# buctcurry/ICKA

Hardware: AMD Instinct MI355X
Metric: MNER samples/sec (fwd+bwd) at seq=128, 36 regions, bs=32 per GPU (higher is better)
Workload: dtype bf16; 1 GPU; c2: bert(H768,L12,h12,I3072)+36x2048 regions, seq_len 128, per-GPU batch 32, 1 cross layer(s), gated head, 13 labels, train mode p=0.1, token-CE loss; global_batch=32, seq_len=128, regions=36, parallelism=dp1, launch=hipgraph, precision=bf16, accumulate=1

## Files before the change

icka_amd/csrc/fusion.hip:

```cpp
#include <math.h>

#include "common.h"

namespace {

__device__ __forceinline__ void ld8(const bf16_t* p, float (&o)[8]) {
    const bf16x8 v = as_bf16x8(*reinterpret_cast<const u32x4*>(p));
#pragma unroll
    for (int e = 0; e < 8; ++e) o[e] = bf2f(v[e]);
}
__device__ __forceinline__ void st8(bf16_t* p, const float (&v)[8]) {
    bf16x8 o;
#pragma unroll
    for (int e = 0; e < 8; ++e) o[e] = f2bf(v[e]);
    *reinterpret_cast<u32x4*>(p) = as_u32x4(o);
}
__device__ __forceinline__ float block_sum(float v, float* red) {
    v = wave_sum(v);
    const int w = threadIdx.x >> 6;
    if ((threadIdx.x & 63) == 0) red[w] = v;
    __syncthreads();
    float t = 0.f;
    for (int i = 0; i < (int)(blockDim.x >> 6); ++i) t += red[i];
    __syncthreads();
// ... 261 lines not shown
                       (const bf16_t*)seq, lds, (const bf16_t*)cross, ldc, dW, dbias, B, S, H, accumulate);
    ICKA_CHECK_LAUNCH();
    return 0;
}


namespace {

constexpr int CLS_TB = 16;
constexpr int CLS_MAXC = 16;

__device__ __forceinline__ void cls_ld8(const bf16_t* p, float (&o)[8]) {
    const bf16x8 v = as_bf16x8(*reinterpret_cast<const u32x4*>(p));
#pragma unroll
    for (int e = 0; e < 8; ++e) o[e] = bf2f(v[e]);
}
__device__ __forceinline__ void cls_st8(bf16_t* p, const float (&v)[8]) {
    bf16x8 o;
#pragma unroll
    for (int e = 0; e < 8; ++e) o[e] = f2bf(v[e]);
    *reinterpret_cast<u32x4*>(p) = as_u32x4(o);
}

template <bool F16>
__global__ __launch_bounds__(256) void cls_head_fwd_kernel(const bf16_t* __restrict__ seq, const bf16_t* __restrict__ gated,
                                                           const bf16_t* __restrict__ W, const float* __restrict__ bias,
                                                           float* __restrict__ logits, int M, int H, int C) {
    extern __shared__ __attribute__((aligned(16))) char cls_smem[];
    __shared__ float s_red[4][CLS_MAXC][65];
    bf16_t* sW = reinterpret_cast<bf16_t*>(cls_smem);
    const int tid = threadIdx.x, lane = tid & 63, wave = tid >> 6;
    const int nch = (2 * H) >> 3, hch = H >> 3;
    for (int i = tid; i < C * nch; i += 256)
        *reinterpret_cast<u32x4*>(sW + (int64_t)i * 8) = *reinterpret_cast<const u32x4*>(W + (int64_t)i * 8);
    __syncthreads();
    const int nw = gridDim.x * 4;
    for (int row0 = (blockIdx.x * 4 + wave) * 2; row0 < M; row0 += 2 * nw) {
        u32x4 xr[2][4];
#pragma unroll
        for (int r = 0; r < 2; ++r)
#pragma unroll
            for (int i = 0; i < 4; ++i) {
                const int j = lane + 64 * i, row = row0 + r;
                xr[r][i] = u32x4{0u, 0u, 0u, 0u};
                if (j < nch && row < M)
                    xr[r][i] = *reinterpret_cast<const u32x4*>(j < hch ? seq + (int64_t)row * H + j * 8
                                                                       : gated + (int64_t)row * H + (j - hch) * 8);
            }
        float acc[2][CLS_MAXC];
#pragma unroll
        for (int r = 0; r < 2; ++r)
#pragma unroll
            for (int c = 0; c < CLS_MAXC; ++c) acc[r][c] = 0.f;
#pragma unroll
        for (int i = 0; i < 4; ++i) {
            const int j = lane + 64 * i;
            if (j < nch) {
#pragma unroll
                for (int c = 0; c < CLS_MAXC; ++c) {
                    if (c < C) {
                        float w[8];
                        if constexpr (F16) {
                            const f16x8 wv = __builtin_bit_cast(f16x8, *reinterpret_cast<const u32x4*>(sW + (int64_t)c * 2 * H + j * 8));
#pragma unroll
                            for (int e = 0; e < 8; ++e) w[e] = (float)wv[e];
                        } else {
                            cls_ld8(sW + (int64_t)c * 2 * H + j * 8, w);
                        }
#pragma unroll
                        for (int r = 0; r < 2; ++r) {
                            if constexpr (F16) {
// ... 94 lines not shown
            } else {
                const bf16x8 gv = as_bf16x8(gr[u]), cv = as_bf16x8(cr4[u]);
                float uu[8], dc[8];
#pragma unroll
                for (int e = 0; e < 8; ++e) {
                    const float g = bf2f(gv[e]);
                    uu[e] = dx[e] * bf2f(cv[e]) * g * (1.f - g);
                    dc[e] = dx[e] * g;
                }
                cls_st8(du + row * H + h, uu);
                cls_st8(dcross + row * H + h, dc);
            }
        }
    }
#pragma unroll
    for (int c = 0; c < CC; ++c)
        if (c < C) {
            float* p = myslab + (int64_t)c * 2 * H + j * 8;
            *reinterpret_cast<f32x4*>(p) = f32x4{dW[c][0], dW[c][1], dW[c][2], dW[c][3]};
            *reinterpret_cast<f32x4*>(p + 4) = f32x4{dW[c][4], dW[c][5], dW[c][6], dW[c][7]};
        }
}

}

extern "C" int32_t icka_cls_head_bwd_slabs(int32_t M) { return (M + CLS_TB - 1) / CLS_TB; }
extern "C" int64_t icka_cls_head_slab_floats(int32_t H, int32_t C) { return (int64_t)C * 2 * H + CLS_MAXC; }

static int cls_head_fwd_impl(bool f16, const void* seq, const void* gated, const void* W, const float* bias, float* logits,
                             int32_t M, int32_t H, int32_t C, void* stream) {
    if (!seq || !gated || !W || !logits) return ICKA_E_ARG;
    if (M <= 0 || H <= 0 || H % 8 || C <= 0 || C > CLS_MAXC || 2 * H / 8 > 256 || (int64_t)C * 2 * H * 2 > 44 * 1024)
        return ICKA_E_SHAPE;
    if ((reinterpret_cast<uintptr_t>(seq) | reinterpret_cast<uintptr_t>(gated) | reinterpret_cast<uintptr_t>(W)) & 15)
        return ICKA_E_ALIGN;
    int grid = (M + 7) / 8;
    grid = grid > 512 ? 512 : grid;
    if (f16)
        hipLaunchKernelGGL(cls_head_fwd_kernel<true>, dim3(grid), dim3(256), (size_t)C * 2 * H * 2, (hipStream_t)stream,
                           (const bf16_t*)seq, (const bf16_t*)gated, (const bf16_t*)W, bias, logits, M, H, C);
    else
        hipLaunchKernelGGL(cls_head_fwd_kernel<false>, dim3(grid), dim3(256), (size_t)C * 2 * H * 2, (hipStream_t)stream,
                           (const bf16_t*)seq, (const bf16_t*)gated, (const bf16_t*)W, bias, logits, M, H, C);
    ICKA_CHECK_LAUNCH();
    return 0;
}
extern "C" int icka_cls_head_fwd(const void* seq, const void* gated, const void* W, const float* bias, float* logits,
                                 int32_t M, int32_t H, int32_t C, void* stream) {
    return cls_head_fwd_impl(false, seq, gated, W, bias, logits, M, H, C, stream);
}
extern "C" int icka_cls_head_fwd_h(const void* seq, const void* gated, const void* W, const float* bias, float* logits,
                                   int32_t M, int32_t H, int32_t C, void* stream) {
    return cls_head_fwd_impl(true, seq, gated, W, bias, logits, M, H, C, stream);
}

extern "C" int icka_cls_head_bwd(const void* dl, int64_t ldd, const void* seq, const void* gated, const void* gate,
                                 const void* cross, const void* W, void* dseq, void* du, void* dcross, float* partials,
                                 int32_t M, int32_t H, int32_t C, void* stream) {
    if (!dl || !seq || !gated || !gate || !cross || !W || !dseq || !du || !dcross || !partials) return ICKA_E_ARG;
    if (M <= 0 || H <= 0 || H % 8 || C <= 0 || C > CLS_MAXC || 2 * H / 8 > 256 || ldd < C) return ICKA_E_SHAPE;
    const uintptr_t al = reinterpret_cast<uintptr_t>(seq) | reinterpret_cast<uintptr_t>(gated) |
                         reinterpret_cast<uintptr_t>(gate) | reinterpret_cast<uintptr_t>(cross) |
                         reinterpret_cast<uintptr_t>(W) | reinterpret_cast<uintptr_t>(dseq) |
                         reinterpret_cast<uintptr_t>(du) | reinterpret_cast<uintptr_t>(dcross) |
                         reinterpret_cast<uintptr_t>(partials);
    if (al & 15) return ICKA_E_ALIGN;
    const int grid = icka_cls_head_bwd_slabs(M);
    if (C <= 13)
        hipLaunchKernelGGL((cls_head_bwd_kernel<13>), dim3(grid), dim3(256), 0, (hipStream_t)stream,
                           (const bf16_t*)dl, ldd, (const bf16_t*)seq, (const bf16_t*)gated, (const bf16_t*)gate,
                           (const bf16_t*)cross, (const bf16_t*)W, (bf16_t*)dseq, (bf16_t*)du, (bf16_t*)dcross,
                           partials, M, H, C);
    else
        hipLaunchKernelGGL((cls_head_bwd_kernel<CLS_MAXC>), dim3(grid), dim3(256), 0, (hipStream_t)stream,
                           (const bf16_t*)dl, ldd, (const bf16_t*)seq, (const bf16_t*)gated, (const bf16_t*)gate,
                           (const bf16_t*)cross, (const bf16_t*)W, (bf16_t*)dseq, (bf16_t*)du, (bf16_t*)dcross,
                           partials, M, H, C);
    ICKA_CHECK_LAUNCH();
    return 0;
}
```

icka_amd/csrc/layernorm.hip:

```cpp
#include "common.h"
#include "ln_row.h"
#include <cstdlib>

namespace {

constexpr int BWD_BLOCKS = 1024;
constexpr int SLOTS = 4;

template <int NCH>
__global__ __launch_bounds__(256) void ln_fwd_kernel(const LnFwdArgs a_) {
    LnFwdArgs a = a_;
    a.drop = drop_resolve(a.drop);
    const int lane = threadIdx.x & 63;
    const int wid = blockIdx.x * 4 + (threadIdx.x >> 6), nw = gridDim.x * 4;
    ln_fwd_rows<NCH>(a, wid, nw, a.M, lane);
}

struct LnBwdArgs {
    const bf16_t* dy; int64_t lddy; const bf16_t* dy2; int64_t lddy2; const bf16_t* xhat; const float* rstd;
    const float* gamma; bf16_t* dres; int64_t lddres; bf16_t* dx; int64_t lddx; float* partials;
    int M, H; DropCfg drop;
    uint8_t* row_live; uint8_t* row_live_kv; const float* add_mask; int mask_S;
};

// ... 192 lines not shown
}
__global__ __launch_bounds__(256) void ln_cols_kernel(const bf16_t* __restrict__ dy, int64_t lddy,
                                                      const bf16_t* __restrict__ dy2, int64_t lddy2,
                                                      const bf16_t* __restrict__ xhat, const bf16_t* __restrict__ dx,
                                                      int64_t lddx, float* __restrict__ partials, int M, int H,
                                                      int rows_per_group) {
    ln_cols_body(dy, lddy, dy2, lddy2, xhat, dx, lddx, partials, M, H, rows_per_group, blockIdx.x, blockIdx.y);
}

struct LnColsArgs {
    int nx, groups, rows_per_group;
};
template <int NCH, bool LIVE = false>
__global__ __launch_bounds__(256) void ln_bwd_fused_kernel(const LnBwdArgs a, const LnColsArgs c) {
    const int ncol = c.nx * c.groups;
    if ((int)blockIdx.x >= ncol) {
        ln_rows_body<NCH, LIVE>(a, blockIdx.x - ncol, gridDim.x - ncol);
        return;
    }
    ln_cols_body(a.dy, a.lddy, a.dy2, a.lddy2, a.xhat, nullptr, 0, a.partials, a.M, a.H, c.rows_per_group,
                 blockIdx.x % c.nx, blockIdx.x / c.nx);
}

__global__ __launch_bounds__(1024) void finalize_kernel(const float* __restrict__ partials, int nslab, int H, float* o0,
                                                        float* o1, float* o2, float* o3, int accumulate) {
    __shared__ float red[16][64];
    const int cx = threadIdx.x & 63, sy = threadIdx.x >> 6;
    const int idx = blockIdx.x * 64 + cx;
    float s = 0.f;
    if (idx < SLOTS * H) {
        const int slot = idx / H, c = idx - slot * H;
        for (int b = sy; b < nslab; b += 16) s += partials[((int64_t)b * SLOTS + slot) * H + c];
    }
    red[sy][cx] = s;
    __syncthreads();
    if (sy == 0 && idx < SLOTS * H) {
        const int slot = idx / H, c = idx - slot * H;
        float* out = slot == 0 ? o0 : slot == 1 ? o1 : slot == 2 ? o2 : o3;
        if (out) {
            float t = 0.f;
#pragma unroll
            for (int k = 0; k < 16; ++k) t += red[k][cx];
            out[c] = accumulate ? out[c] + t : t;
        }
    }
}

struct EmbFwdArgs {
    const int64_t* ids; const int64_t* tt; const float* word; const float* pos; const float* type;
    const float* gamma; const float* beta; bf16_t* y; void* yf; bf16_t* xhat; float* rstd;
    int M, S, H, vocab, n_type; float eps; DropCfg drop;
    const int32_t* src; const bf16_t* prompt; int S_in, P, pos_offset;
    int yf_f16;
};

template <int NCH>
__global__ __launch_bounds__(256) void embed_fwd_kernel(const EmbFwdArgs a_) {
    EmbFwdArgs a = a_;
    a.drop = drop_resolve(a.drop);
    const int lane = threadIdx.x & 63;
    const int wid = blockIdx.x * 4 + (threadIdx.x >> 6), nw = gridDim.x * 4;
    const int nchunk = a.H >> 3;
    const float inv_h = 1.f / (float)a.H;
    for (int row = wid; row < a.M; row += nw) {
        const int sp = row % a.S;
        const int sidx = a.src ? a.src[sp] : sp;
        const bf16_t* prow = sidx < 0 ? a.prompt + ((int64_t)(row / a.S) * a.P + (-1 - sidx)) * a.H : nullptr;
// ... 36 lines not shown
                float g[8], b[8], xh[8], o[8];
                load8f(a.gamma + c * 8, g);
                load8f(a.beta + c * 8, b);
                const uint32_t base = (uint32_t)row * (uint32_t)a.H + c * 8;
#pragma unroll
                for (int e = 0; e < 8; ++e) {
                    xh[e] = (s[i][e] - mean) * rstd;
                    o[e] = (g[e] * xh[e] + b[e]) * drop_mul(a.drop, base + e);
                }
                store8(a.y + (int64_t)row * a.H + c * 8, o);
                if (a.yf) store8t(a.yf, a.yf_f16, (int64_t)row * a.H + c * 8, o);
                if (a.xhat) store8(a.xhat + (int64_t)row * a.H + c * 8, xh);
            }
        }
    }
}

struct EmbBwdArgs {
    const bf16_t* dy; const int64_t* ids; const int64_t* tt; const bf16_t* xhat; const float* rstd;
    const float* gamma; float* dword; float* dpos; float* dtype; float* partials;
    int M, S, H, vocab, n_type, padding_idx; DropCfg drop;
    const int32_t* src; bf16_t* dprompt; int S_in, P, pos_offset;
    float* dtok;
};

template <int NCH>
__global__ __launch_bounds__(256) void embed_bwd_kernel(const EmbBwdArgs a_) {
    EmbBwdArgs a = a_;
    a.drop = drop_resolve(a.drop);
    extern __shared__ __attribute__((aligned(16))) float lds_f[];
    const int lane = threadIdx.x & 63;
    const int wid = blockIdx.x * 4 + (threadIdx.x >> 6), nw = gridDim.x * 4;
    const int nchunk = a.H >> 3;
    const float inv_h = 1.f / (float)a.H;
    float acc[4][NCH][8];
#pragma unroll
    for (int s = 0; s < 4; ++s)
#pragma unroll
        for (int i = 0; i < NCH; ++i)
#pragma unroll
            for (int e = 0; e < 8; ++e) acc[s][i][e] = 0.f;

    for (int row = wid; row < a.M; row += nw) {
        int64_t id = a.ids[row];
        id = id < 0 ? 0 : (id >= a.vocab ? a.vocab - 1 : id);
        int64_t t = a.tt ? a.tt[row] : 0;
// ... 38 lines not shown
                    }
                }
            }
        }
        __builtin_amdgcn_wave_barrier();
        for (int j = lane; j < a.H; j += 64) {
            const float ds = rowbuf[j];
            if (a.dtok) a.dtok[(int64_t)row * a.H + j] = id != a.padding_idx ? ds : 0.f;
            else if (id != a.padding_idx) atomicAdd(a.dword + id * a.H + j, ds);
            atomicAdd(a.dpos + (int64_t)sp * a.H + j, ds);
            if (a.n_type > 2) atomicAdd(a.dtype + t * a.H + j, ds);
        }
        __builtin_amdgcn_wave_barrier();
    }
    flush_columns<NCH, 4>(acc, lds_f, a.partials, a.H);
}

template <int NCH>
__global__ __launch_bounds__(512) void embed_bwd_pos_kernel(const EmbBwdArgs a_) {
    EmbBwdArgs a = a_;
    a.drop = drop_resolve(a.drop);
    extern __shared__ __attribute__((aligned(16))) float lds_f[];
    const int tid = threadIdx.x, lane = tid & 63, wave = tid >> 6;
    const int sp = blockIdx.x, B = a.M / a.S;
    const int nchunk = a.H >> 3;
    const float inv_h = 1.f / (float)a.H;
    float acc[5][NCH][8];
#pragma unroll
    for (int s = 0; s < 5; ++s)
#pragma unroll
        for (int i = 0; i < NCH; ++i)
#pragma unroll
            for (int e = 0; e < 8; ++e) acc[s][i][e] = 0.f;
    float* rowbuf = lds_f + wave * a.H;

    const int sidx = a.src ? a.src[sp] : sp;
    for (int b = wave; b < B; b += 8) {
        const int row = b * a.S + sp;
        int64_t id = sidx < 0 ? 0 : a.ids[a.src ? (int64_t)b * a.S_in + sidx : row];
        id = id < 0 ? 0 : (id >= a.vocab ? a.vocab - 1 : id);
        int64_t t = a.tt ? a.tt[row] : 0;
        t = t < 0 ? 0 : (t >= a.n_type ? a.n_type - 1 : t);
        float xh[NCH][8], gd[NCH][8];
        float s1 = 0.f, s2 = 0.f;
#pragma unroll
        for (int i = 0; i < NCH; ++i) {
            const int c = lane + 64 * i;
            if (c < nchunk) {
                float dy[8], g[8];
                load8(a.dy + (int64_t)row * a.H + c * 8, dy);
                load8(a.xhat + (int64_t)row * a.H + c * 8, xh[i]);
                load8f(a.gamma + c * 8, g);
                const uint32_t base = (uint32_t)row * (uint32_t)a.H + c * 8;
#pragma unroll
                for (int e = 0; e < 8; ++e) {
                    const float dl = dy[e] * drop_mul(a.drop, base + e);
                    gd[i][e] = g[e] * dl;
                    s1 += gd[i][e];
                    s2 += gd[i][e] * xh[i][e];
                    acc[0][i][e] += dl * xh[i][e];
// ... 32 lines not shown
                const float ds = rowbuf[j];
                if (id != a.padding_idx) atomicAdd(a.dword + id * a.H + j, ds);
                if (a.n_type > 2) atomicAdd(a.dtype + t * a.H + j, ds);
            }
        }
        __builtin_amdgcn_wave_barrier();
    }
#pragma unroll
    for (int s = 0; s < 5; ++s) {
        __syncthreads();
#pragma unroll
        for (int i = 0; i < NCH; ++i) {
            const int c = lane + 64 * i;
            if (c < nchunk) {
#pragma unroll
                for (int e = 0; e < 8; ++e) rowbuf[c * 8 + e] = acc[s][i][e];
            }
        }
        __syncthreads();
        for (int j = tid; j < a.H; j += 512) {
            float v = 0.f;
#pragma unroll
            for (int w = 0; w < 8; ++w) v += lds_f[w * a.H + j];
            if (s < 4) a.partials[((int64_t)sp * SLOTS + s) * a.H + j] = v;
            else a.dpos[(int64_t)(sp + a.pos_offset) * a.H + j] += v;
        }
    }
}

inline int pick_nch(int H) { return (H / 8 + 63) / 64; }
inline int rows_knob(const char* name, int dflt) {
    const char* e = getenv(name);
    const int v = e ? atoi(e) : 0;
    return v >= 1 && v <= 16 ? v : dflt;
}
const int kLnRowsEnv = rows_knob("ICKA_TUNE_LN_ROWS_PER_WAVE", 0);
const int kLnBwdRowsEnv = rows_knob("ICKA_TUNE_LN_BWD_ROWS_PER_WAVE", 1);
inline int row_grid(int M) { int g = (M + 3) / 4; return g > 2048 ? 2048 : (g < 1 ? 1 : g); }
inline int fwd_grid(int M) {
    const int r = kLnRowsEnv ? kLnRowsEnv : (M >= 4096 ? 2 : 1);
    int g = (M + 4 * r - 1) / (4 * r);
    return g > 2048 ? 2048 : (g < 1 ? 1 : g);
}
inline int bwd_grid(int M) { int g = (M + 3) / 4; return g > BWD_BLOCKS ? BWD_BLOCKS : (g < 1 ? 1 : g); }
inline int bwd_row_grid(int M) {
    const int r = kLnBwdRowsEnv;
    int g = (M + 4 * r - 1) / (4 * r);
    return g > 2048 ? 2048 : (g < 1 ? 1 : g);
}
inline bool al16(const void* p) { return (reinterpret_cast<uintptr_t>(p) & 15) == 0; }

#define DISPATCH_NCH(nch, KERNEL, grid, shmem, st, args)                                                 \
    switch (nch) {                                                                                       \
        case 1: hipLaunchKernelGGL((KERNEL<1>), dim3(grid), dim3(256), shmem, st, args); break;          \
        case 2: hipLaunchKernelGGL((KERNEL<2>), dim3(grid), dim3(256), shmem, st, args); break;          \
        case 3: hipLaunchKernelGGL((KERNEL<3>), dim3(grid), dim3(256), shmem, st, args); break;          \
        default: hipLaunchKernelGGL((KERNEL<4>), dim3(grid), dim3(256), shmem, st, args); break;         \
    }

}
// ... 191 lines not shown
    hipStream_t st = (hipStream_t)stream;
    DISPATCH_NCH(pick_nch(H), embed_fwd_kernel, row_grid(B * S), 0, st, a);
    ICKA_CHECK_LAUNCH();
    return 0;
}

static int embed_bwd_impl(const void* dy, const int64_t* ids, const int64_t* token_type, const void* xhat,
                          const float* rstd, const float* gamma, float* dword, float* dtok, float* dpos, float* dtype,
                          float* dgamma, float* dbeta, float* partials, int32_t B, int32_t S, int32_t H,
                          int32_t vocab, int32_t n_type, int32_t padding_idx, float p_drop, uint64_t seed,
                          int32_t accumulate, void* stream) {
    if (!dy || !ids || !xhat || !rstd || !gamma || (!dword && !dtok) || !dpos || !dtype || !dgamma || !dbeta || !partials)
        return ICKA_E_ARG;
    if (B <= 0 || S <= 0 || H <= 0 || H % 8 != 0 || H > 8 * 64 * MAX_CH || vocab <= 0 || n_type <= 0)
        return ICKA_E_SHAPE;
    if (!al16(dy) || !al16(xhat) || !al16(gamma)) return ICKA_E_ALIGN;
    EmbBwdArgs a{(const bf16_t*)dy, ids, token_type, (const bf16_t*)xhat, rstd, gamma, dword, dpos, dtype, partials,
                 B * S, S, H, vocab, n_type, padding_idx, make_drop(p_drop, seed), nullptr, nullptr, S, 0, 0, dtok};
    hipStream_t st = (hipStream_t)stream;
    if (n_type > 2 && !accumulate &&
        hipMemsetAsync(dtype, 0, sizeof(float) * (size_t)n_type * H, st) != hipSuccess)
        return ICKA_E_ARG;
    int grid = bwd_grid(B * S);
    if (S <= BWD_BLOCKS) {
        grid = S;
        switch (pick_nch(H)) {
            case 1: hipLaunchKernelGGL((embed_bwd_pos_kernel<1>), dim3(S), dim3(512), 8 * H * sizeof(float), st, a); break;
            case 2: hipLaunchKernelGGL((embed_bwd_pos_kernel<2>), dim3(S), dim3(512), 8 * H * sizeof(float), st, a); break;
            case 3: hipLaunchKernelGGL((embed_bwd_pos_kernel<3>), dim3(S), dim3(512), 8 * H * sizeof(float), st, a); break;
            default: hipLaunchKernelGGL((embed_bwd_pos_kernel<4>), dim3(S), dim3(512), 8 * H * sizeof(float), st, a); break;
        }
    } else {
        DISPATCH_NCH(pick_nch(H), embed_bwd_kernel, grid, 8 * H * sizeof(float), st, a);
    }
    ICKA_CHECK_LAUNCH();
    float* t0 = n_type <= 2 ? dtype : nullptr;
    float* t1 = n_type == 2 ? dtype + H : nullptr;
    hipLaunchKernelGGL(finalize_kernel, dim3((SLOTS * H + 63) / 64), dim3(1024), 0, st, partials, grid, H, dgamma,
                       dbeta, t0, t1, accumulate);
    ICKA_CHECK_LAUNCH();
    return 0;
}

extern "C" int icka_embed_bwd(const void* dy, const int64_t* ids, const int64_t* token_type, const void* xhat,
                              const float* rstd, const float* gamma, float* dword, float* dpos, float* dtype,
                              float* dgamma, float* dbeta, float* partials, int32_t B, int32_t S, int32_t H,
                              int32_t vocab, int32_t n_type, int32_t padding_idx, float p_drop, uint64_t seed,
                              int32_t accumulate, void* stream) {
    if (!dword) return ICKA_E_ARG;
    return embed_bwd_impl(dy, ids, token_type, xhat, rstd, gamma, dword, nullptr, dpos, dtype, dgamma, dbeta, partials, B, S, H, vocab,
                          n_type, padding_idx, p_drop, seed, accumulate, stream);
}
extern "C" int icka_embed_bwd_rows(const void* dy, const int64_t* ids, const int64_t* token_type, const void* xhat,
                                   const float* rstd, const float* gamma, float* dtok, float* dpos, float* dtype,
                                   float* dgamma, float* dbeta, float* partials, int32_t B, int32_t S, int32_t H,
                                   int32_t vocab, int32_t n_type, int32_t padding_idx, float p_drop, uint64_t seed,
                                   int32_t accumulate, void* stream) {
    if (!dtok) return ICKA_E_ARG;
    return embed_bwd_impl(dy, ids, token_type, xhat, rstd, gamma, nullptr, dtok, dpos, dtype, dgamma, dbeta, partials, B, S, H, vocab,
                          n_type, padding_idx, p_drop, seed, accumulate, stream);
}

// ... 62 lines not shown
```

icka_amd/ops.py:

```python
from __future__ import annotations

from typing import Optional

import torch

from . import kernels as K
from .arena import ParamArena
from .attention_maps import current as _maps_recorder

BF16, F32, F16 = torch.bfloat16, torch.float32, torch.float16
import os as _os
ATTN_KEEPBITS = _os.environ.get("ICKA_ATTN_KEEPBITS", "auto")
FUSE_DENSE_LN = _os.environ.get("ICKA_FUSE_DENSE_LN", "1") != "0"
FUSE_DENSE_LN_MIN_ROWS = 3072
FUSE_QKV_ATTN = _os.environ.get("ICKA_FUSE_QKV_ATTN", "1") != "0"
FUSE_QKV_ATTN_MIN_ROWS = 3072
WGRAD_LIVE = _os.environ.get("ICKA_WGRAD_LIVE", "1") != "0"


def _keepbits_on(Sq: int, Skv: int) -> bool:
    if ATTN_KEEPBITS == "auto":
        return Sq > 128 and Skv > 128 and Sq <= 256 and Skv <= 256
    return ATTN_KEEPBITS == "1"


def _empty(ref: torch.Tensor, *shape, dtype=BF16) -> torch.Tensor:
    return torch.empty(*shape, dtype=dtype, device=ref.device)


def _c(t: torch.Tensor) -> torch.Tensor:
    if t.dtype != BF16:
        raise TypeError("expected a bf16 gradient, got %s" % t.dtype)
    return t if t.is_contiguous() else t.contiguous()


class Dims(object):
    __slots__ = ("B", "S", "R", "H", "I", "heads", "eps", "p_hidden", "p_attn", "train", "h16", "pack")

    def __init__(self, B, S, R, H, I, heads, eps, p_hidden, p_attn, train, h16=False, pack=None):
        self.B, self.S, self.R, self.H, self.I, self.heads, self.eps = B, S, R, H, I, heads, eps
# ... 199 lines not shown
            K.attn_bwd_packed(q, k, v, add_mask, dctx, lse, delta, dqkv[:, :H], dqkv[:, H:2 * H], dqkv[:, 2 * H:], d.pack.cu,
                              True, d.B, d.heads, d.S, Skv, p_drop=d.p_attn, seed=seed_a, keepbits=kb)
        else:
            K.attn_bwd(q, k, v, add_mask, ctx, dctx, lse, delta, dqkv[:, :H], dqkv[:, H:2 * H], dqkv[:, 2 * H:], d.B,
                       d.heads, d.S, Skv, p_drop=d.p_attn, seed=seed_a, keepbits=kb)
        wg = (sa.query.weight, sa.key.weight, sa.value.weight)
        bg = (sa.query.bias, sa.key.bias, sa.value.bias)
        _wgrad(A, dqkv, x, A.g_cat(wg), A.grad_beta(wg), bias=bg, k_live=k_live)
        dx = _empty(x, M, H)
        K.gemm(K.GEMM_NN, dqkv, A.w_cat(wg), dx, **epi)
        return dx, None
    dq = _empty(x, M, H)
    dkv = _empty(x, kv_src.shape[0], 2 * H)
    if kv_src.shape[0] > d.B * Skv:
        K.zero_rows_(dkv, d.B * Skv)
    if generic:
        _attn_generic_bwd(lse, False, dctx, d, Skv, seed_a, dq, dkv)
    elif d.pack is not None:
        K.attn_bwd_packed(qkv, kvbuf[:, :H], kvbuf[:, H:], add_mask, dctx, lse, delta, dq, dkv[:, :H], dkv[:, H:], d.pack.cu,
                          False, d.B, d.heads, d.S, Skv, p_drop=d.p_attn, seed=seed_a, keepbits=kb)
    else:
        K.attn_bwd(qkv, kvbuf[:, :H], kvbuf[:, H:], add_mask, ctx, dctx, lse, delta, dq, dkv[:, :H], dkv[:, H:], d.B,
                   d.heads, d.S, Skv, p_drop=d.p_attn, seed=seed_a, keepbits=kb)
    _wgrad(A, dq, x, A.g(sa.query.weight), A.grad_beta(sa.query.weight), bias=sa.query.bias)
    wg = (sa.key.weight, sa.value.weight)
    bg = (sa.key.bias, sa.value.bias)
    _wgrad(A, dkv, kv_src, A.g_cat(wg), A.grad_beta(wg), bias=bg)
    dx = _empty(x, M, H)
    K.gemm(K.GEMM_NN, dq, A.w(sa.query.weight), dx, **epi)
    dsrc = None
    if need_dkv_src:
        dsrc = _empty(x, kv_src.shape[0], H)
        K.gemm(K.GEMM_NN, dkv, A.w_cat(wg), dsrc)
    return dx, dsrc


def _dense_norm_fwd(A: ParamArena, mod, h, res, d: Dims, save: bool, h16=None):
    M = h.shape[0]
    H = mod.dense.weight.shape[0]
    o = _empty(h, M, H, dtype=F32)
    y = _empty(h, M, H)
    yf = _empty(h, M, H, dtype=F16 if d.h16 else F32)
    xhat = _empty(h, M, H) if save else None
    rstd = _empty(h, M, dtype=F32) if save else None
    seed_h = A.next_seed() if d.p_hidden > 0 else 0
    twin = {"y_f16": yf} if d.h16 else {"y_f32": yf}
    if FUSE_DENSE_LN and h16 is None and M >= FUSE_DENSE_LN_MIN_ROWS:
# ... 38 lines not shown


def _inter_bwd(A: ParamArena, inter, x, dz, dres, k_live=None):
    _wgrad(A, dz, x, A.g(inter.dense.weight), A.grad_beta(inter.dense.weight), bias=inter.dense.bias, k_live=k_live)
    dx = _empty(x, x.shape[0], x.shape[1])
    if dres is not None:
        K.gemm(K.GEMM_NN, dz, A.w(inter.dense.weight), dx, epilogue=K.EPI_ADD, aux=dres)
    else:
        K.gemm(K.GEMM_NN, dz, A.w(inter.dense.weight), dx)
    return dx


def _attn_block_fwd(A: ParamArena, att, x, xres, kv_src, add_mask, d: Dims, Skv: int, save: bool, kv16=None):
    xres = _fwd_twin(A, x, xres, d)
    ctx, ctx16, s_core = _attn_core_fwd(A, att.self, x, kv_src, add_mask, d, Skv, save, x16=xres if d.h16 else None,
                                        kv16=kv16 if d.h16 else None)
    y, yf, s_out = _dense_norm_fwd(A, att.output, ctx, x if xres is None else xres, d, save, h16=ctx16)
    return y, yf, ((ctx, s_core, s_out) if save else None)


def _attn_block_bwd(A: ParamArena, att, x, kv_src, add_mask, d: Dims, Skv: int, saved, dy, dy2, need_dkv_src: bool,
                    live=False):
    ctx, s_core, s_out = saved
    live = live and kv_src is None
    dao, dres, flags = _dense_norm_bwd(A, "ln_attn", att.output, ctx, d, s_out, dy, dy2, live=live,
                                       add_mask=add_mask if live else None)
    dctx = _empty(x, x.shape[0], x.shape[1])
    K.gemm(K.GEMM_NN, dao, A.w(att.output.dense.weight), dctx)
    return _attn_core_bwd(A, att.self, x, kv_src, add_mask, d, Skv, s_core, ctx, dctx, dres, need_dkv_src,
                          k_live=flags[1] if flags else None)


def _ffn_block_fwd(A: ParamArena, layer, x, xres, d: Dims, save: bool):
    xres = _fwd_twin(A, x, xres, d)
    g, z, g16 = _inter_fwd(A, layer.intermediate, x, xres if d.h16 else None)
    y, yf, s_out = _dense_norm_fwd(A, layer.output, g, x if xres is None else xres, d, save, h16=g16)
    return y, yf, ((z, g, s_out) if save else None)


def _ffn_block_bwd(A: ParamArena, layer, x, d: Dims, saved, dy, dy2=None, live=False):
    z, g, s_out = saved
    dfo, dres, flags = _dense_norm_bwd(A, "ln_ffn", layer.output, g, d, s_out, dy, dy2, live=live)
    dz = _empty(x, z.shape[0], z.shape[1])
    K.gemm(K.GEMM_NN, dfo, A.w(layer.output.dense.weight), dz, epilogue=K.EPI_DGELU, aux=z)
    return _inter_bwd(A, layer.intermediate, x, dz, dres, k_live=flags[0] if flags else None)


class EmbeddingsFn(torch.autograd.Function):

    @staticmethod
    def forward(ctx, anchor, mod, A: ParamArena, ids, tt, d: Dims):
        B, S = ids.shape
        H = d.H
# ... 68 lines not shown
        _flush_wgrad(A)
        A.flush_final()
        return None, dx, None, None, None, None, None


class CrossLayerFn(torch.autograd.Function):

    @staticmethod
    def forward(ctx, anchor, s1, s1f, s2, layer, A: ParamArena, add_mask, d: Dims, s2_16=None):
        save = any(ctx.needs_input_grad)
        x1, x1f, s_att = _attn_block_fwd(A, layer.attention, s1, s1f, s2, add_mask, d, d.R, save, kv16=s2_16)
        x2, x2f, s_ffn = _ffn_block_fwd(A, layer, x1, x1f, d, save)
        ctx.layer, ctx.A, ctx.d, ctx.s_att, ctx.s_ffn = layer, A, d, s_att, s_ffn
        ctx.need_s2 = s2.requires_grad
        ctx.save_for_backward(s1, s2, x1, add_mask)
        ctx.mark_non_differentiable(x2f)
        ctx.set_materialize_grads(False)
        return x2, x2f

    @staticmethod
    def backward(ctx, dy, _dyf=None):
        s1, s2, x1, add_mask = ctx.saved_tensors
        layer, A, d = ctx.layer, ctx.A, ctx.d
        dx1 = _ffn_block_bwd(A, layer, x1, d, ctx.s_ffn, _c(dy))
        ds1, ds2 = _attn_block_bwd(A, layer.attention, s1, s2, add_mask, d, d.R, ctx.s_att, dx1, None, ctx.need_s2)
        if not A.keep_saved:
            ctx.s_att = ctx.s_ffn = None
        _flush_wgrad(A)
        A.flush_final()
        return None, ds1, None, ds2, None, None, None, None, None


class AttnCoreFn(torch.autograd.Function):

    @staticmethod
    def forward(ctx, anchor, x, kv_src, sa, A: ParamArena, add_mask, d: Dims, Skv: int):
        save = any(ctx.needs_input_grad)
        c, _c16, saved = _attn_core_fwd(A, sa, x, kv_src, add_mask, d, Skv, save)
        ctx.sa, ctx.A, ctx.d, ctx.Skv, ctx.saved = sa, A, d, Skv, saved
        ctx.need_kv = kv_src is not None and kv_src.requires_grad
        ctx.save_for_backward(x, kv_src, add_mask, c)
        return c

    @staticmethod
    def backward(ctx, dc):
        x, kv_src, add_mask, c = ctx.saved_tensors
        A = ctx.A
        dx, dsrc = _attn_core_bwd(A, ctx.sa, x, kv_src, add_mask, ctx.d, ctx.Skv, ctx.saved, c, _c(dc), None, ctx.need_kv)
# ... 531 lines not shown
```

Baseline: 7120 samples/s.

## Widen cls head kernels, split embed bwd over batch, enable live wgrad in cross layer

```diff
diff --git a/icka_amd/csrc/fusion.hip b/icka_amd/csrc/fusion.hip
--- a/icka_amd/csrc/fusion.hip
+++ b/icka_amd/csrc/fusion.hip
@@ -307,31 +307,39 @@
     *reinterpret_cast<u32x4*>(p) = as_u32x4(o);
 }
 
-template <bool F16>
-__global__ __launch_bounds__(256) void cls_head_fwd_kernel(const bf16_t* __restrict__ seq, const bf16_t* __restrict__ gated,
-                                                           const bf16_t* __restrict__ W, const float* __restrict__ bias,
-                                                           float* __restrict__ logits, int M, int H, int C) {
+__device__ __forceinline__ void cls_fwd_ld_rows(const bf16_t* __restrict__ seq, const bf16_t* __restrict__ gated, int row0,
+                                                int lane, int M, int H, u32x4 (&xr)[2][4]) {
+    const int nch = (2 * H) >> 3, hch = H >> 3;
+#pragma unroll
+    for (int r = 0; r < 2; ++r)
+#pragma unroll
+        for (int i = 0; i < 4; ++i) {
+            const int j = lane + 64 * i, row = row0 + r;
+            xr[r][i] = u32x4{0u, 0u, 0u, 0u};
+            if (j < nch && row < M)
+                xr[r][i] = *reinterpret_cast<const u32x4*>(j < hch ? seq + (int64_t)row * H + j * 8
+                                                                   : gated + (int64_t)row * H + (j - hch) * 8);
+        }
+}
+
+template <bool F16, int NW>
+__global__ __launch_bounds__(NW * 64) void cls_head_fwd_kernel(const bf16_t* __restrict__ seq, const bf16_t* __restrict__ gated,
+                                                               const bf16_t* __restrict__ W, const float* __restrict__ bias,
+                                                               float* __restrict__ logits, int M, int H, int C) {
     extern __shared__ __attribute__((aligned(16))) char cls_smem[];
-    __shared__ float s_red[4][CLS_MAXC][65];
+    __shared__ float s_red[NW][CLS_MAXC][65];
     bf16_t* sW = reinterpret_cast<bf16_t*>(cls_smem);
     const int tid = threadIdx.x, lane = tid & 63, wave = tid >> 6;
-    const int nch = (2 * H) >> 3, hch = H >> 3;
-    for (int i = tid; i < C * nch; i += 256)
+    const int nch = (2 * H) >> 3;
+    const int nw = gridDim.x * NW;
+    const int first = (blockIdx.x * NW + wave) * 2;
+    u32x4 xr[2][4];
+    if constexpr (NW == 8) cls_fwd_ld_rows(seq, gated, first, lane, M, H, xr);
+    for (int i = tid; i < C * nch; i += NW * 64)
         *reinterpret_cast<u32x4*>(sW + (int64_t)i * 8) = *reinterpret_cast<const u32x4*>(W + (int64_t)i * 8);
     __syncthreads();
-    const int nw = gridDim.x * 4;
-    for (int row0 = (blockIdx.x * 4 + wave) * 2; row0 < M; row0 += 2 * nw) {
-        u32x4 xr[2][4];
-#pragma unroll
-        for (int r = 0; r < 2; ++r)
-#pragma unroll
-            for (int i = 0; i < 4; ++i) {
-                const int j = lane + 64 * i, row = row0 + r;
-                xr[r][i] = u32x4{0u, 0u, 0u, 0u};
-                if (j < nch && row < M)
-                    xr[r][i] = *reinterpret_cast<const u32x4*>(j < hch ? seq + (int64_t)row * H + j * 8
-                                                                       : gated + (int64_t)row * H + (j - hch) * 8);
-            }
+    for (int row0 = first; row0 < M; row0 += 2 * nw) {
+        if (NW != 8 || row0 != first) cls_fwd_ld_rows(seq, gated, row0, lane, M, H, xr);
         float acc[2][CLS_MAXC];
 #pragma unroll
         for (int r = 0; r < 2; ++r)
@@ -472,7 +480,104 @@
         }
 }
 
-}
+__device__ __forceinline__ void cls_ld4(const bf16_t* p, float (&o)[4]) {
+    const bf16x4 v = __builtin_bit_cast(bf16x4, *reinterpret_cast<const u32x2*>(p));
+#pragma unroll
+    for (int e = 0; e < 4; ++e) o[e] = bf2f(v[e]);
+}
+__device__ __forceinline__ void cls_st4(bf16_t* p, const float (&v)[4]) {
+    bf16x4 o;
+#pragma unroll
+    for (int e = 0; e < 4; ++e) o[e] = f2bf(v[e]);
+    *reinterpret_cast<u32x2*>(p) = __builtin_bit_cast(u32x2, o);
+}
+
+template <int CC>
+__global__ __launch_bounds__(512) void cls_head_bwd4_kernel(const bf16_t* __restrict__ dl, int64_t ldd,
+                                                            const bf16_t* __restrict__ seq, const bf16_t* __restrict__ gated,
+                                                            const bf16_t* __restrict__ gate, const bf16_t* __restrict__ cross,
+                                                            const bf16_t* __restrict__ W, bf16_t* __restrict__ dseq,
+                                                            bf16_t* __restrict__ du, bf16_t* __restrict__ dcross,
+                                                            float* __restrict__ partials, int M, int H, int C) {
+    __shared__ float s_dl[CLS_TB][CLS_MAXC];
+    const int tid = threadIdx.x;
+    const int nq = (2 * H) >> 2, hq = H >> 2;
+    const int t0 = blockIdx.x * CLS_TB;
+    const int nt = M - t0 < CLS_TB ? M - t0 : CLS_TB;
+    for (int i = tid; i < CLS_TB * CLS_MAXC; i += blockDim.x) {
+        const int t = i / CLS_MAXC, c = i % CLS_MAXC;
+        s_dl[t][c] = (t < nt && c < C) ? bf2f(dl[(int64_t)(t0 + t) * ldd + c]) : 0.f;
+    }
+    __syncthreads();
+    const int64_t slab = (int64_t)C * 2 * H + CLS_MAXC;
+    float* myslab = partials + (int64_t)blockIdx.x * slab;
+    if (tid < CLS_MAXC) {
+        float s = 0.f;
+        for (int t = 0; t < nt; ++t) s += s_dl[t][tid];
+        myslab[(int64_t)C * 2 * H + tid] = s;
+    }
+    const int j = tid;
+    if (j >= nq) return;
+    const bool second = j >= hq;
+    const int h = (second ? j - hq : j) * 4;
+    float Wr[CC][4], dW[CC][4];
+#pragma unroll
+    for (int c = 0; c < CC; ++c) {
+        if (c < C) cls_ld4(W + (int64_t)c * 2 * H + j * 4, Wr[c]);
+#pragma unroll
+        for (int e = 0; e < 4; ++e) { dW[c][e] = 0.f; if (c >= C) Wr[c][e] = 0.f; }
+    }
+    for (int tb = 0; tb < nt; tb += 8) {
+        u32x2 xr[8], gr[8], cr8[8];
+#pragma unroll
+        for (int u = 0; u < 8; ++u) {
+            const int64_t row = t0 + (tb + u < nt ? tb + u : nt - 1);
+            xr[u] = *reinterpret_cast<const u32x2*>((second ? gated : seq) + row * H + h);
+            if (second) {
+                gr[u] = *reinterpret_cast<const u32x2*>(gate + row * H + h);
+                cr8[u] = *reinterpret_cast<const u32x2*>(cross + row * H + h);
+            }
+        }
+#pragma unroll
+        for (int u = 0; u < 8; ++u) {
+            const int t = tb + u;
+            if (t >= nt) break;
+            const int64_t row = t0 + t;
+            const bf16x4 xv = __builtin_bit_cast(bf16x4, xr[u]);
+            float x[4], dx[4];
+#pragma unroll
+            for (int e = 0; e < 4; ++e) { x[e] = bf2f(xv[e]); dx[e] = 0.f; }
+#pragma unroll
+            for (int c = 0; c < CC; ++c) {
+                const float d = s_dl[t][c];
+#pragma unroll
+                for (int e = 0; e < 4; ++e) { dx[e] += d * Wr[c][e]; dW[c][e] += d * x[e]; }
+            }
+            if (!second) {
+                cls_st4(dseq + row * H + h, dx);
+            } else {
+                const bf16x4 gv = __builtin_bit_cast(bf16x4, gr[u]), cv = __builtin_bit_cast(bf16x4, cr8[u]);
+                float uu[4], dc[4];
+#pragma unroll
+                for (int e = 0; e < 4; ++e) {
+                    const float g = bf2f(gv[e]);
+                    uu[e] = dx[e] * bf2f(cv[e]) * g * (1.f - g);
+                    dc[e] = dx[e] * g;
+                }
+                cls_st4(du + row * H + h, uu);
+                cls_st4(dcross + row * H + h, dc);
+            }
+        }
+    }
+#pragma unroll
+    for (int c = 0; c < CC; ++c)
+        if (c < C)
+            *reinterpret_cast<f32x4*>(myslab + (int64_t)c * 2 * H + j * 4) = f32x4{dW[c][0], dW[c][1], dW[c][2], dW[c][3]};
+}
+
+}
+
+static const bool kClsHeadWide = !(getenv("ICKA_CLS_HEAD_WIDE") && atoi(getenv("ICKA_CLS_HEAD_WIDE")) == 0);
 
 extern "C" int32_t icka_cls_head_bwd_slabs(int32_t M) { return (M + CLS_TB - 1) / CLS_TB; }
 extern "C" int64_t icka_cls_head_slab_floats(int32_t H, int32_t C) { return (int64_t)C * 2 * H + CLS_MAXC; }
@@ -484,13 +589,25 @@
         return ICKA_E_SHAPE;
     if ((reinterpret_cast<uintptr_t>(seq) | reinterpret_cast<uintptr_t>(gated) | reinterpret_cast<uintptr_t>(W)) & 15)
         return ICKA_E_ALIGN;
+    if (kClsHeadWide) {
+        int grid = (M + 15) / 16;
+        grid = grid > 256 ? 256 : grid;
+        if (f16)
+            hipLaunchKernelGGL((cls_head_fwd_kernel<true, 8>), dim3(grid), dim3(512), (size_t)C * 2 * H * 2, (hipStream_t)stream,
+                               (const bf16_t*)seq, (const bf16_t*)gated, (const bf16_t*)W, bias, logits, M, H, C);
+        else
+            hipLaunchKernelGGL((cls_head_fwd_kernel<false, 8>), dim3(grid), dim3(512), (size_t)C * 2 * H * 2, (hipStream_t)stream,
+                               (const bf16_t*)seq, (const bf16_t*)gated, (const bf16_t*)W, bias, logits, M, H, C);
+        ICKA_CHECK_LAUNCH();
+        return 0;
+    }
     int grid = (M + 7) / 8;
     grid = grid > 512 ? 512 : grid;
     if (f16)
-        hipLaunchKernelGGL(cls_head_fwd_kernel<true>, dim3(grid), dim3(256), (size_t)C * 2 * H * 2, (hipStream_t)stream,
+        hipLaunchKernelGGL((cls_head_fwd_kernel<true, 4>), dim3(grid), dim3(256), (size_t)C * 2 * H * 2, (hipStream_t)stream,
                            (const bf16_t*)seq, (const bf16_t*)gated, (const bf16_t*)W, bias, logits, M, H, C);
     else
-        hipLaunchKernelGGL(cls_head_fwd_kernel<false>, dim3(grid), dim3(256), (size_t)C * 2 * H * 2, (hipStream_t)stream,
+        hipLaunchKernelGGL((cls_head_fwd_kernel<false, 4>), dim3(grid), dim3(256), (size_t)C * 2 * H * 2, (hipStream_t)stream,
                            (const bf16_t*)seq, (const bf16_t*)gated, (const bf16_t*)W, bias, logits, M, H, C);
     ICKA_CHECK_LAUNCH();
     return 0;
@@ -516,6 +633,21 @@
                          reinterpret_cast<uintptr_t>(partials);
     if (al & 15) return ICKA_E_ALIGN;
     const int grid = icka_cls_head_bwd_slabs(M);
+    if (kClsHeadWide) {
+        const int threads = (2 * H / 4 + 63) / 64 * 64;
+        if (C <= 13)
+            hipLaunchKernelGGL((cls_head_bwd4_kernel<13>), dim3(grid), dim3(threads), 0, (hipStream_t)stream,
+                               (const bf16_t*)dl, ldd, (const bf16_t*)seq, (const bf16_t*)gated, (const bf16_t*)gate,
+                               (const bf16_t*)cross, (const bf16_t*)W, (bf16_t*)dseq, (bf16_t*)du, (bf16_t*)dcross,
+                               partials, M, H, C);
+        else
+            hipLaunchKernelGGL((cls_head_bwd4_kernel<CLS_MAXC>), dim3(grid), dim3(threads), 0, (hipStream_t)stream,
+                               (const bf16_t*)dl, ldd, (const bf16_t*)seq, (const bf16_t*)gated, (const bf16_t*)gate,
+                               (const bf16_t*)cross, (const bf16_t*)W, (bf16_t*)dseq, (bf16_t*)du, (bf16_t*)dcross,
+                               partials, M, H, C);
+        ICKA_CHECK_LAUNCH();
+        return 0;
+    }
     if (C <= 13)
         hipLaunchKernelGGL((cls_head_bwd_kernel<13>), dim3(grid), dim3(256), 0, (hipStream_t)stream,
                            (const bf16_t*)dl, ldd, (const bf16_t*)seq, (const bf16_t*)gated, (const bf16_t*)gate,
diff --git a/icka_amd/csrc/layernorm.hip b/icka_amd/csrc/layernorm.hip
--- a/icka_amd/csrc/layernorm.hip
+++ b/icka_amd/csrc/layernorm.hip
@@ -238,15 +238,25 @@
                  blockIdx.x % c.nx, blockIdx.x / c.nx);
 }
 
-__global__ __launch_bounds__(1024) void finalize_kernel(const float* __restrict__ partials, int nslab, int H, float* o0,
-                                                        float* o1, float* o2, float* o3, int accumulate) {
+__device__ __forceinline__ void finalize_body(const float* __restrict__ partials, int nslab, int H, float* o0, float* o1,
+                                              float* o2, float* o3, int accumulate, int bx) {
     __shared__ float red[16][64];
     const int cx = threadIdx.x & 63, sy = threadIdx.x >> 6;
-    const int idx = blockIdx.x * 64 + cx;
+    const int idx = bx * 64 + cx;
     float s = 0.f;
     if (idx < SLOTS * H) {
         const int slot = idx / H, c = idx - slot * H;
-        for (int b = sy; b < nslab; b += 16) s += partials[((int64_t)b * SLOTS + slot) * H + c];
+        const float* p = partials + (int64_t)slot * H + c;
+        const int64_t st = (int64_t)SLOTS * H;
+        int b = sy;
+        for (; b + 48 < nslab; b += 64) {
+            const float v0 = p[b * st], v1 = p[(b + 16) * st], v2 = p[(b + 32) * st], v3 = p[(b + 48) * st];
+            s += v0;
+            s += v1;
+            s += v2;
+            s += v3;
+        }
+        for (; b < nslab; b += 16) s += p[b * st];
     }
     red[sy][cx] = s;
     __syncthreads();
@@ -259,6 +269,27 @@
             for (int k = 0; k < 16; ++k) t += red[k][cx];
             out[c] = accumulate ? out[c] + t : t;
         }
+    }
+}
+
+__global__ __launch_bounds__(1024) void finalize_kernel(const float* __restrict__ partials, int nslab, int H, float* o0,
+                                                        float* o1, float* o2, float* o3, int accumulate) {
+    finalize_body(partials, nslab, H, o0, o1, o2, o3, accumulate, blockIdx.x);
+}
+
+__global__ __launch_bounds__(1024) void embed_finalize_kernel(const float* __restrict__ partials, int nslab, int H, float* o0,
+                                                              float* o1, float* o2, float* o3, int accumulate, int ncol,
+                                                              const float* __restrict__ dpos_part, float* __restrict__ dpos,
+                                                              int n, int nsplit) {
+    if ((int)blockIdx.x < ncol) {
+        finalize_body(partials, nslab, H, o0, o1, o2, o3, accumulate, blockIdx.x);
+        return;
+    }
+    const int i = ((int)blockIdx.x - ncol) * 1024 + threadIdx.x;
+    if (i < n) {
+        float t = dpos_part[i];
+        for (int h = 1; h < nsplit; ++h) t += dpos_part[(int64_t)h * n + i];
+        dpos[i] += t;
     }
 }
 
@@ -341,6 +372,7 @@
     int M, S, H, vocab, n_type, padding_idx; DropCfg drop;
     const int32_t* src; bf16_t* dprompt; int S_in, P, pos_offset;
     float* dtok;
+    int nsplit; float* dpos_part;
 };
 
 template <int NCH>
@@ -425,7 +457,11 @@
     a.drop = drop_resolve(a.drop);
     extern __shared__ __attribute__((aligned(16))) float lds_f[];
     const int tid = threadIdx.x, lane = tid & 63, wave = tid >> 6;
-    const int sp = blockIdx.x, B = a.M / a.S;
+    const int B = a.M / a.S;
+    const int nsplit = a.nsplit > 1 ? a.nsplit : 1;
+    const int part = (int)blockIdx.x / a.S, sp = (int)blockIdx.x - part * a.S;
+    const int bper = (B + nsplit - 1) / nsplit;
+    const int b_end = (part + 1) * bper < B ? (part + 1) * bper : B;
     const int nchunk = a.H >> 3;
     const float inv_h = 1.f / (float)a.H;
     float acc[5][NCH][8];
@@ -438,7 +474,7 @@
     float* rowbuf = lds_f + wave * a.H;
 
     const int sidx = a.src ? a.src[sp] : sp;
-    for (int b = wave; b < B; b += 8) {
+    for (int b = part * bper + wave; b < b_end; b += 8) {
         const int row = b * a.S + sp;
         int64_t id = sidx < 0 ? 0 : a.ids[a.src ? (int64_t)b * a.S_in + sidx : row];
         id = id < 0 ? 0 : (id >= a.vocab ? a.vocab - 1 : id);
@@ -517,7 +553,8 @@
             float v = 0.f;
 #pragma unroll
             for (int w = 0; w < 8; ++w) v += lds_f[w * a.H + j];
-            if (s < 4) a.partials[((int64_t)sp * SLOTS + s) * a.H + j] = v;
+            if (s < 4) a.partials[((int64_t)blockIdx.x * SLOTS + s) * a.H + j] = v;
+            else if (nsplit > 1) a.dpos_part[(int64_t)blockIdx.x * a.H + j] = v;
             else a.dpos[(int64_t)(sp + a.pos_offset) * a.H + j] += v;
         }
     }
@@ -531,6 +568,7 @@
 }
 const int kLnRowsEnv = rows_knob("ICKA_TUNE_LN_ROWS_PER_WAVE", 0);
 const int kLnBwdRowsEnv = rows_knob("ICKA_TUNE_LN_BWD_ROWS_PER_WAVE", 1);
+const bool kEmbedBwdSplit = !(getenv("ICKA_EMBED_BWD_SPLIT") && atoi(getenv("ICKA_EMBED_BWD_SPLIT")) == 0);
 inline int row_grid(int M) { int g = (M + 3) / 4; return g > 2048 ? 2048 : (g < 1 ? 1 : g); }
 inline int fwd_grid(int M) {
     const int r = kLnRowsEnv ? kLnRowsEnv : (M >= 4096 ? 2 : 1);
@@ -768,13 +806,16 @@
         hipMemsetAsync(dtype, 0, sizeof(float) * (size_t)n_type * H, st) != hipSuccess)
         return ICKA_E_ARG;
     int grid = bwd_grid(B * S);
+    const int nsplit = kEmbedBwdSplit && 2 * S <= 256 && B >= 2 ? 2 : 1;
+    float* dpos_part = partials + (int64_t)nsplit * S * SLOTS * H;
     if (S <= BWD_BLOCKS) {
-        grid = S;
+        grid = nsplit * S;
+        if (nsplit > 1) { a.nsplit = nsplit; a.dpos_part = dpos_part; }
         switch (pick_nch(H)) {
-            case 1: hipLaunchKernelGGL((embed_bwd_pos_kernel<1>), dim3(S), dim3(512), 8 * H * sizeof(float), st, a); break;
-            case 2: hipLaunchKernelGGL((embed_bwd_pos_kernel<2>), dim3(S), dim3(512), 8 * H * sizeof(float), st, a); break;
-            case 3: hipLaunchKernelGGL((embed_bwd_pos_kernel<3>), dim3(S), dim3(512), 8 * H * sizeof(float), st, a); break;
-            default: hipLaunchKernelGGL((embed_bwd_pos_kernel<4>), dim3(S), dim3(512), 8 * H * sizeof(float), st, a); break;
+            case 1: hipLaunchKernelGGL((embed_bwd_pos_kernel<1>), dim3(grid), dim3(512), 8 * H * sizeof(float), st, a); break;
+            case 2: hipLaunchKernelGGL((embed_bwd_pos_kernel<2>), dim3(grid), dim3(512), 8 * H * sizeof(float), st, a); break;
+            case 3: hipLaunchKernelGGL((embed_bwd_pos_kernel<3>), dim3(grid), dim3(512), 8 * H * sizeof(float), st, a); break;
+            default: hipLaunchKernelGGL((embed_bwd_pos_kernel<4>), dim3(grid), dim3(512), 8 * H * sizeof(float), st, a); break;
         }
     } else {
         DISPATCH_NCH(pick_nch(H), embed_bwd_kernel, grid, 8 * H * sizeof(float), st, a);
@@ -782,8 +823,12 @@
     ICKA_CHECK_LAUNCH();
     float* t0 = n_type <= 2 ? dtype : nullptr;
     float* t1 = n_type == 2 ? dtype + H : nullptr;
-    hipLaunchKernelGGL(finalize_kernel, dim3((SLOTS * H + 63) / 64), dim3(1024), 0, st, partials, grid, H, dgamma,
-                       dbeta, t0, t1, accumulate);
+    const int ncol = (SLOTS * H + 63) / 64;
+    if (a.nsplit > 1)
+        hipLaunchKernelGGL(embed_finalize_kernel, dim3(ncol + (S * H + 1023) / 1024), dim3(1024), 0, st, partials, grid, H,
+                           dgamma, dbeta, t0, t1, accumulate, ncol, dpos_part, dpos, S * H, nsplit);
+    else
+        hipLaunchKernelGGL(finalize_kernel, dim3(ncol), dim3(1024), 0, st, partials, grid, H, dgamma, dbeta, t0, t1, accumulate);
     ICKA_CHECK_LAUNCH();
     return 0;
 }
diff --git a/icka_amd/ops.py b/icka_amd/ops.py
--- a/icka_amd/ops.py
+++ b/icka_amd/ops.py
@@ -16,6 +16,7 @@
 FUSE_QKV_ATTN = _os.environ.get("ICKA_FUSE_QKV_ATTN", "1") != "0"
 FUSE_QKV_ATTN_MIN_ROWS = 3072
 WGRAD_LIVE = _os.environ.get("ICKA_WGRAD_LIVE", "1") != "0"
+CROSS_WGRAD_LIVE = _os.environ.get("ICKA_CROSS_WGRAD_LIVE", "1") != "0"
 
 
 def _keepbits_on(Sq: int, Skv: int) -> bool:
@@ -261,7 +262,7 @@
     else:
         K.attn_bwd(qkv, kvbuf[:, :H], kvbuf[:, H:], add_mask, ctx, dctx, lse, delta, dq, dkv[:, :H], dkv[:, H:], d.B,
                    d.heads, d.S, Skv, p_drop=d.p_attn, seed=seed_a, keepbits=kb)
-    _wgrad(A, dq, x, A.g(sa.query.weight), A.grad_beta(sa.query.weight), bias=sa.query.bias)
+    _wgrad(A, dq, x, A.g(sa.query.weight), A.grad_beta(sa.query.weight), bias=sa.query.bias, k_live=k_live)
     wg = (sa.key.weight, sa.value.weight)
     bg = (sa.key.bias, sa.value.bias)
     _wgrad(A, dkv, kv_src, A.g_cat(wg), A.grad_beta(wg), bias=bg)
@@ -346,13 +347,13 @@
 def _attn_block_bwd(A: ParamArena, att, x, kv_src, add_mask, d: Dims, Skv: int, saved, dy, dy2, need_dkv_src: bool,
                     live=False):
     ctx, s_core, s_out = saved
-    live = live and kv_src is None
+    cross = kv_src is not None
     dao, dres, flags = _dense_norm_bwd(A, "ln_attn", att.output, ctx, d, s_out, dy, dy2, live=live,
-                                       add_mask=add_mask if live else None)
+                                       add_mask=add_mask if live and not cross else None)
     dctx = _empty(x, x.shape[0], x.shape[1])
     K.gemm(K.GEMM_NN, dao, A.w(att.output.dense.weight), dctx)
     return _attn_core_bwd(A, att.self, x, kv_src, add_mask, d, Skv, s_core, ctx, dctx, dres, need_dkv_src,
-                          k_live=flags[1] if flags else None)
+                          k_live=flags[0 if cross else 1] if flags else None)
 
 
 def _ffn_block_fwd(A: ParamArena, layer, x, xres, d: Dims, save: bool):
@@ -467,8 +468,9 @@
     def backward(ctx, dy, _dyf=None):
         s1, s2, x1, add_mask = ctx.saved_tensors
         layer, A, d = ctx.layer, ctx.A, ctx.d
-        dx1 = _ffn_block_bwd(A, layer, x1, d, ctx.s_ffn, _c(dy))
-        ds1, ds2 = _attn_block_bwd(A, layer.attention, s1, s2, add_mask, d, d.R, ctx.s_att, dx1, None, ctx.need_s2)
+        live = WGRAD_LIVE and CROSS_WGRAD_LIVE and d.pack is None
+        dx1 = _ffn_block_bwd(A, layer, x1, d, ctx.s_ffn, _c(dy), live=live)
+        ds1, ds2 = _attn_block_bwd(A, layer.attention, s1, s2, add_mask, d, d.R, ctx.s_att, dx1, None, ctx.need_s2, live=live)
         if not A.keep_saved:
             ctx.s_att = ctx.s_ffn = None
         _flush_wgrad(A)
```

New measurement: 7179 samples/s, median of 6. No clear change (+0.8%).
